# colopl/libpoporon

Measured on AMD Instinct MI355X. Metric: RS(255,223) codewords/s (encode; decode @ t=16 errs) and GB/s vs HBM peak, 1/2/4/8 GPU, higher is better.
Workload: dtype u8; 1 GPU; RS(255,223) round trip: encode + decode with 16 errors per codeword, 1048576 codewords per GPU (BASELINE configs[1]+[2]); codewords_per_gpu=1048576, layout=255-byte codeword rows, stride 255, code=poporon_config_rs_default (8, 0x11D, fcr 1, prim 1, 32 roots)

## Files before the change

### libpoporon_amd/csrc/rs_fast.hip

```cpp
#include <hip/hip_runtime.h>

#include <type_traits>

#include "rs_device.h"
#include "rs_gfa.h"
#include "rs_lane.h"

#define FWG 1024
#define NL 17
#define BWG 512
#define BM_WAVES 4

#define FAST_ROUNDS 8
static int fast_grid(size_t count, int num_cu)
{
    const size_t need = (count + FWG - 1) / FWG;
    const size_t g = FAST_ROUNDS * 2u * (size_t)(num_cu > 0 ? num_cu : 256);
    return (int)(need < g ? (need ? need : 1) : g);
}


template <bool NRG>
__global__ __launch_bounds__(BWG, BM_WAVES) void rs_bm_k(const RsDevTables *__restrict__ T, const uint8_t *__restrict__ syn,
                                                   size_t count, uint8_t *__restrict__ lamo, uint8_t *__restrict__ omo,
                                                   uint8_t *__restrict__ meta, uint32_t *__restrict__ list,
                                                   uint32_t *__restrict__ nlist, uint8_t *__restrict__ ok,
                                                   uint8_t *__restrict__ corrected, uint32_t npar)
{
    __shared__ uint32_t lgf[512 * 32];
    fill_gfa<BWG>(lgf, T);
    __syncthreads();
    const GfA gf{lds_addr(lgf) + 4u * (threadIdx.x & 31u) + 1u};
    const uint32_t pofs = gf.pofs;
    const uint32_t AZ = gf.az();
    constexpr uint32_t DQZ = SZ;

    for (size_t base = (size_t)blockIdx.x * BWG; base < count; base += (size_t)gridDim.x * BWG) {
        const size_t cw = base + threadIdx.x;
        const bool valid = cw < count;
        const uint32_t *sp = reinterpret_cast<const uint32_t *>(syn + (valid ? cw : 0) * RS_NR);
        uint4 sa = make_uint4(0, 0, 0, 0), sb = sa;
        if (valid) {
            sa = reinterpret_cast<const uint4 *>(sp)[0];
            sb = reinterpret_cast<const uint4 *>(sp)[1];
        }
        const bool any = (sa.x | sa.y | sa.z | sa.w | sb.x | sb.y | sb.z | sb.w) != 0u;
        if (__ballot(any) == 0ull) {
            if (valid) {
                ok[cw] = 1;
                if (corrected)
                    corrected[cw] = 0;
                meta[cw] = (uint8_t)(RS_ST_DONE << 5);
            }
            continue;
        }

        const uint32_t HZ = pofs + 1u;
        uint32_t hl[NL], B[NL + 1];
        hl[0] = HZ + 128u;
#pragma unroll
        for (int i = 1; i < NL; ++i)
            hl[i] = HZ;
        B[0] = pofs;
#pragma unroll
        for (int k = 1; k <= NL; ++k)
            B[k] = AZ;
        uint32_t dl = 0, db = 0, L = 0, lb = 0, ubp = 0;
        uint32_t over = 0, bo = 0;
        uint32_t WL[20];
#pragma unroll
        for (int k = 0; k < 20; ++k)
            WL[k] = SZ;
        uint32_t snext = any ? sa.x : 0u;

        auto step = [&](auto sc, uint32_t r) __attribute__((always_inline)) {
            constexpr int s = decltype(sc)::value;
            const uint32_t ub = ubp;
            uint32_t la[NL];
            uint32_t disc = 0;
            la[0] = pofs;
#pragma unroll
            for (int g = 0; g < NL; g += 4) {
#pragma unroll
                for (int i = g; i < g + 4 && i < NL; ++i)
                    if (i > 0)
                        la[i] = AZ;
                if ((uint32_t)g <= ub) {
#pragma unroll
                    for (int i = g; i < g + 4 && i < NL; ++i) {
                        if (i > 0)
                            la[i] = lds16(hl[i]);
                        disc ^= gf.expa(la[i] + WL[3 - s + i]);
                    }
                }
            }
            const uint32_t ld = gf.logs(disc);
            const bool upd = disc != 0u;
            const bool lengthen = upd && (2u * L <= r - 1u);
            const int32_t dd = (int32_t)ld - (int32_t)lb;
            const uint32_t dq = upd ? (uint32_t)(dd < 0 ? dd + 255 * 128 : dd) : DQZ;
            const uint32_t b16 = B[NL - 1] != AZ;
            over |= upd ? (bo | b16) : 0u;
            bo = lengthen ? 0u : (bo | b16);
            const uint32_t up = min((uint32_t)(NL - 1), max(dl, db + 1u));
            const uint32_t ub2 = wave_max_full(up);
            ubp = ub2;
            const uint64_t lmask = __ballot(lengthen);
            static_for<0, (NL - 1) / 4 + 1, 1>([&](auto mc) __attribute__((always_inline)) {
                constexpr int m = (NL - 1) / 4 - decltype(mc)::value;
                if ((uint32_t)(4 * m) <= ub2) {
#pragma unroll
                    for (int i = 4 * m + 3; i >= 4 * m; --i)
                        if (i > 0 && i < NL)
                            hl[i] ^= shl7(gf.expa(dq + B[i - 1]));
                    if constexpr (4 * m + 3 < NL) {
                        const uint32_t b0 = m > 0 ? B[m > 0 ? 4 * m - 1 : 0] : AZ;
                        asm("s_mov_b64 vcc, %8\n\t"
                            "v_cndmask_b32_e32 %3, %2, %7, vcc\n\t"
                            "v_cndmask_b32_e32 %2, %1, %6, vcc\n\t"
                            "v_cndmask_b32_e32 %1, %0, %5, vcc\n\t"
                            "v_cndmask_b32_e32 %0, %9, %4, vcc"
                            : "+v"(B[4 * m]), "+v"(B[4 * m + 1]), "+v"(B[4 * m + 2]), "+v"(B[4 * m + 3])
                            : "v"(la[4 * m]), "v"(la[4 * m + 1]), "v"(la[4 * m + 2]), "v"(la[4 * m + 3]),
                              "s"(lmask), "v"(b0)
                            : "vcc");
                    } else {
                        B[4 * m] = lengthen ? la[4 * m] : B[4 * m - 1];
                    }
                }
            });
            db = lengthen ? dl : min(db + 1u, (uint32_t)(NL - 1));
            if (upd)
                dl = up;
            if (lengthen) {
                L = r - L;
                lb = ld;
            }
        };
        const uint32_t nq = NRG ? (npar + 3u) >> 2 : RS_NR / 4;
#pragma unroll 1
        for (uint32_t q = 0; q < nq; ++q) {
            const uint32_t sd = snext;
            if (q + 1u < nq)
                snext = any ? sp[q + 1u] : 0u;
            const uint32_t s0 = gf.logs(sd & 0xffu), s1 = gf.logs((sd >> 8) & 0xffu);
            const uint32_t s2 = gf.logs((sd >> 16) & 0xffu), s3 = gf.logs(sd >> 24);
#pragma unroll
            for (int k = 19; k >= 4; --k)
                WL[k] = WL[k - 4];
            WL[0] = s3, WL[1] = s2, WL[2] = s1, WL[3] = s0;
            step(std::integral_constant<int, 0>{}, 4u * q + 1u);
            if (!NRG || 4u * q + 2u <= npar)
                step(std::integral_constant<int, 1>{}, 4u * q + 2u);
            if (!NRG || 4u * q + 3u <= npar)
                step(std::integral_constant<int, 2>{}, 4u * q + 3u);
            if (!NRG || 4u * q + 4u <= npar)
                step(std::integral_constant<int, 3>{}, 4u * q + 4u);
        }

        uint32_t al[NL];
        al[0] = pofs;
#pragma unroll
        for (int i = 1; i < NL; ++i)
            al[i] = (uint32_t)i <= ubp ? lds16(hl[i]) : AZ;
        uint32_t deg = 0;
#pragma unroll
        for (int i = 0; i < NL; ++i)
            deg = (al[i] & 1u) ? (uint32_t)i : deg;
        const bool fast = any && !over && deg == L && deg != 0u && (!NRG || 2u * L <= npar);

        uint32_t ob[4] = {0xFFFFFFFFu, 0xFFFFFFFFu, 0xFFFFFFFFu, 0xFFFFFFFFu};
        const uint32_t degmax = wave_max(fast ? deg : 0u);
        if (degmax) {
            const uint4 s4 = any ? reinterpret_cast<const uint4 *>(sp)[0] : make_uint4(0, 0, 0, 0);
            const uint32_t sw[4] = {s4.x, s4.y, s4.z, s4.w};
            auto omega = [&](auto dmc) __attribute__((always_inline)) {
                constexpr int DM = decltype(dmc)::value;
                uint32_t sl[16];
#pragma unroll
                for (int k = 0; k < 16; ++k)
                    sl[k] = gf.logs((sw[k >> 2] >> (8 * (k & 3))) & 0xffu);
#pragma unroll
                for (int m = 0; m < 16; ++m) {
                    if (DM ? m < DM : (uint32_t)m < degmax) {
                        uint32_t acc = 0;
#pragma unroll
                        for (int j = 0; j <= m; ++j)
                            acc ^= gf.expa(al[j] + sl[m - j]);
                        const uint32_t o = (uint32_t)m < deg ? gf.plog(gf.loga(acc)) : 255u;
                        ob[m >> 2] ^= (o ^ 0xffu) << (8 * (m & 3));
                    }
                    __builtin_amdgcn_sched_barrier(0);
                }
            };
            if (degmax == 16u)
                omega(std::integral_constant<int, 16>{});
            else
                omega(std::integral_constant<int, 0>{});
        }

        if (valid) {
            if (!any) {
                ok[cw] = 1;
                if (corrected)
                    corrected[cw] = 0;
                meta[cw] = (uint8_t)(RS_ST_DONE << 5);
            } else if (!fast) {
                meta[cw] = (uint8_t)(RS_ST_LIST << 5);
                list[atomicAdd(nlist, 1u)] = (uint32_t)cw;
            } else {
                uint32_t lb4[4] = {0, 0, 0, 0};
#pragma unroll
                for (int j = 1; j < NL; ++j)
                    lb4[(j - 1) >> 2] |= gf.plog(al[j]) << (8 * ((j - 1) & 3));
                reinterpret_cast<uint4 *>(lamo)[cw] = make_uint4(lb4[0], lb4[1], lb4[2], lb4[3]);
                reinterpret_cast<uint4 *>(omo)[cw] = make_uint4(ob[0], ob[1], ob[2], ob[3]);
                meta[cw] = (uint8_t)((RS_ST_FAST << 5) | deg);
            }
        }
    }
}




__device__ __forceinline__ uint32_t root_point(uint32_t e)
{
    return (e & 0xE0u) + 28u + ((e >> 3) & 3u) - 4u * (e & 7u);
}

__global__ __launch_bounds__(FWG, 8) void rs_chien_k(const RsDevTables *__restrict__ T, RsCorrParams P, size_t count,
                                                      const uint8_t *__restrict__ lam, uint8_t *__restrict__ meta,
                                                      uint8_t *__restrict__ roots, uint8_t *__restrict__ ok,
                                                      uint8_t *__restrict__ corrected)
{
    __shared__ uint4 lch[256 * 16];
    __shared__ uint4 lroot[FWG];
    {
        constexpr int K = 256 * 16 / FWG;
        uint4 v[K];
#pragma unroll
        for (int k = 0; k < K; ++k) {
            const uint32_t t = threadIdx.x + k * FWG;
            v[k] = T->chien[(t & 15u) * 256u + (t >> 4)];
        }
#pragma unroll
        for (int k = 0; k < K; ++k)
            lch[threadIdx.x + k * FWG] = v[k];
    }
    __syncthreads();
    const uint32_t cb = lds_addr(lch);
    const uint32_t lr0 = threadIdx.x & 15u;
    constexpr uint32_t WRAP = 255u * 256u;

    for (size_t base = (size_t)blockIdx.x * FWG; base < count; base += (size_t)gridDim.x * FWG) {
        const size_t cw = base + threadIdx.x;
        const bool valid = cw < count;
        const uint32_t st = valid ? meta[cw] : 0u;
        const bool fast = (st >> 5) == RS_ST_FAST;
        if (__ballot(fast) == 0ull)
            continue;
        const uint32_t deg = fast ? (st & 31u) : 0u;
        uint4 l4 = make_uint4(0xFFFFFFFFu, 0xFFFFFFFFu, 0xFFFFFFFFu, 0xFFFFFFFFu);
        if (fast)
            l4 = reinterpret_cast<const uint4 *>(lam)[cw];
        uint32_t lr = lr0;
        asm volatile("" : "+v"(lr));
        uint32_t D[4] = {l4.x, l4.y, l4.z, l4.w};
        uint32_t E[4];
#pragma unroll
        for (int k = 0; k < 4; ++k)
            E[k] = (lr & 4u) ? D[(k + 1) & 3] : D[k];
#pragma unroll
        for (int k = 0; k < 4; ++k)
            D[k] = (lr & 8u) ? E[(k + 2) & 3] : E[k];
        uint32_t R[4];
#pragma unroll
        for (int k = 0; k < 4; ++k)
            R[k] = __builtin_amdgcn_alignbyte(D[(k + 1) & 3], D[k], lr & 3u);
        uint32_t A[16], inc[16];
#pragma unroll
        for (int k = 0; k < 16; ++k) {
            const uint32_t jm = ((uint32_t)k + lr) & 15u;
            const uint32_t e = (R[k >> 2] >> (8 * (k & 3))) & 0xffu;
            A[k] = cb + (e << 8) + (jm << 4);
            inc[k] = e == 255u ? WRAP : (jm == 15u ? 256u : (jm + 1u) << 12);
        }
        lroot[threadIdx.x] = make_uint4(0, 0, 0, 0);
        uint32_t lp = lds_addr(lroot) + 16u * threadIdx.x;
        uint32_t cnt = 0, z0 = 0;
        auto push = [&](uint32_t v) __attribute__((always_inline)) {
            lds_st8(lp, v);
            lp += 1u;
        };
#pragma unroll 1
        for (int w = 0; w < 8; ++w) {
            uint32_t word = 0;
#pragma unroll
            for (int h = 0; h < 2; ++h) {
                uint32_t acc[4] = {0x01010101u, 0x01010101u, 0x01010101u, 0x01010101u};
#pragma unroll
                for (int k = 0; k < 16; k += 2) {
                    const lds_u32x4_t r1 = lds128(A[k]), r2 = lds128(A[k + 1]);
                    A[k] = chien_step<WRAP>(A[k], inc[k]);
                    A[k + 1] = chien_step<WRAP>(A[k + 1], inc[k + 1]);
                    acc[0] = xor3(acc[0], r1.x, r2.x);
                    acc[1] = xor3(acc[1], r1.y, r2.y);
                    acc[2] = xor3(acc[2], r1.z, r2.z);
                    acc[3] = xor3(acc[3], r1.w, r2.w);
                }
#pragma unroll
                for (int d = 0; d < 4; ++d)
                    word = __builtin_amdgcn_bitop3_b32(word, zero80(acc[d]) >> (d + 4 * h), 0u, 0xF0 | 0xCC);
            }
            if (w == 7)
                word &= ~(1u << 24);
            if (w == 0) {
                z0 = (word >> 7) & 1u;
                word &= ~0x80u;
            }
            cnt += __popc(word);
            const uint32_t wb = 32u * (uint32_t)w;
            while (word != 0u) {
                const uint32_t b = __builtin_ctz(word);
                word &= word - 1u;
                push(wb | b);
            }
        }
        if (z0)
            push(248u);
        cnt += z0;
        const uint4 l4r = lroot[threadIdx.x];
        const uint32_t L[4] = {l4r.x, l4r.y, l4r.z, l4r.w};
        bool good = cnt == deg;
        if (P.pad > 0) {
            bool low = false;
#pragma unroll
            for (int n = 0; n < 16; ++n) {
                const uint32_t i = root_point((L[n >> 2] >> (8 * (n & 3))) & 0xffu);
                low |= (uint32_t)n < cnt && (int32_t)((i * P.iprim + 254u) % 255u) < P.pad;
            }
            good = good && !low;
        }
        if (fast)
            reinterpret_cast<uint4 *>(roots)[2 * cw] = make_uint4(L[0], L[1], L[2], L[3]);
        if (fast && !good) {
            {
                ok[cw] = 0;
                if (corrected)
                    corrected[cw] = 0;
                meta[cw] = (uint8_t)(RS_ST_DONE << 5);
            }
        }
    }
}


#ifndef F2WG
#define F2WG 1024
#endif
#ifndef F2_WAVES
#define F2_WAVES (F2WG / 128)
#endif
#ifndef FORNEY_R
#define FORNEY_R 2
#endif
template <bool P11>
__global__ __launch_bounds__(F2WG, F2_WAVES) void rs_forney_k(const RsDevTables *__restrict__ T, RsCorrParams P,
                                                      uint8_t *data, size_t dstride, uint8_t *parity, size_t pstride,
                                                      size_t count, const uint8_t *__restrict__ lam,
                                                      const uint8_t *__restrict__ om, uint8_t *__restrict__ roots,
                                                      const uint8_t *__restrict__ meta, uint8_t *__restrict__ ok,
                                                      uint8_t *__restrict__ corrected)
{
    __shared__ uint32_t lgf[512 * 32];
    fill_gfa<F2WG>(lgf, T);
    __syncthreads();
    const GfA gf{lds_addr(lgf) + 4u * (threadIdx.x & 31u) + 1u};
    const int32_t pad = P.pad;
    constexpr bool fcr1 = P11, iprim1 = P11;
    constexpr int R = FORNEY_R;
    const uint32_t mp = 255u * 128u + gf.pofs;

    for (size_t base = (size_t)blockIdx.x * F2WG; base < count; base += (size_t)gridDim.x * F2WG) {
        const size_t cw = base + threadIdx.x;
        const bool valid = cw < count;
        const uint32_t st = valid ? meta[cw] : 0u;
        const bool fast = (st >> 5) == RS_ST_FAST;
        if (__ballot(fast) == 0ull)
            continue;
        const uint32_t deg = fast ? (st & 31u) : 0u;
        uint4 o4 = make_uint4(0xFFFFFFFFu, 0xFFFFFFFFu, 0xFFFFFFFFu, 0xFFFFFFFFu), l4 = o4;
        uint32_t rl[4] = {0, 0, 0, 0};
        if (fast) {
            o4 = reinterpret_cast<const uint4 *>(om)[cw];
            l4 = reinterpret_cast<const uint4 *>(lam)[cw];
            const uint4 ra = reinterpret_cast<const uint4 *>(roots)[2 * cw];
            rl[0] = ra.x, rl[1] = ra.y, rl[2] = ra.z, rl[3] = ra.w;
        }
        const uint32_t ow[4] = {o4.x, o4.y, o4.z, o4.w}, lw[4] = {l4.x, l4.y, l4.z, l4.w};
        const uint32_t dtop = deg ? (deg - 1u) & ~1u : 0u;
        uint32_t opu[16], lod[8];
#pragma unroll
        for (int m = 0; m < 16; ++m)
            opu[m] = gf.afrom((ow[m >> 2] >> (8 * (m & 3))) & 0xffu);
#pragma unroll
        for (int h = 0; h < 8; ++h)
            lod[h] = (uint32_t)(2 * h) <= dtop ? gf.afrom((lw[(2 * h) >> 2] >> (8 * ((2 * h) & 3))) & 0xffu) : gf.az();
        const uint32_t degmax = wave_max(deg);
        uint32_t posp[4] = {0, 0, 0, 0}, magp[4] = {0, 0, 0, 0};
        uint32_t fixed = 0;
#pragma unroll
        for (int n0 = 0; n0 < 16; n0 += R) {
            if ((uint32_t)n0 >= degmax)
                continue;
            uint32_t ir[R], si[R], s[R], num[R], den[R], nh[R], dh[R];
#pragma unroll
            for (int t = 0; t < R; ++t) {
                ir[t] = root_point((rl[(n0 + t) >> 2] >> (8 * ((n0 + t) & 3))) & 0xffu);
                si[t] = 128u * (ir[t] == 255u ? 0u : ir[t]);
                s[t] = num[t] = den[t] = nh[t] = dh[t] = 0;
            }
#pragma unroll
            for (int b = 0; b < 8; ++b) {
#pragma unroll
                for (int t = 0; t < R; ++t) {
                    num[t] ^= gf.expa(opu[b] + s[t]);
                    nh[t] ^= gf.expa(opu[b + 8] + s[t]);
                    if ((b & 1) == 0) {
                        den[t] ^= gf.expa(lod[b >> 1] + s[t]);
                        dh[t] ^= gf.expa(lod[(b >> 1) + 4] + s[t]);
                    }
                    s[t] = addmod7(s[t], si[t]);
                }
                if (b & 1) {
#pragma unroll
                    for (int t = 0; t < R; ++t)
                        asm volatile("" : "+v"(num[t]), "+v"(den[t]), "+v"(nh[t]), "+v"(dh[t]));
                    __builtin_amdgcn_sched_barrier(0);
                }
            }
#pragma unroll
            for (int t = 0; t < R; ++t) {
                num[t] ^= gf.expa(gf.loga(nh[t]) + s[t]);
                den[t] ^= gf.expa(gf.loga(dh[t]) + s[t]);
                uint32_t mag;
                if constexpr (fcr1) {
                    mag = gf.expa(gf.loga(num[t]) - gf.loga(den[t]) + mp);
                } else {
                    const uint32_t ln2 = mod255((uint32_t)((int32_t)ir[t] * ((int32_t)P.fcr - 1) + (int32_t)RS_NN));
                    const uint32_t lden = gf.plog(gf.loga(den[t]));
                    mag = gf.exp(red(gf.plog(gf.loga(num[t])) + ln2 + RS_NN - lden));
                }
                const bool z = (uint32_t)(n0 + t) < deg && num[t] != 0u;
                fixed += z ? 1u : 0u;
                const uint32_t k = iprim1 ? ir[t] - 1u : (ir[t] * P.iprim + 254u) % 255u;
                const uint32_t p = (uint32_t)((int32_t)k - pad);
                posp[(n0 + t) >> 2] |= (p & 0xffu) << (8 * ((n0 + t) & 3));
                magp[(n0 + t) >> 2] |= (z ? mag : 0u) << (8 * ((n0 + t) & 3));
            }
            __builtin_amdgcn_sched_barrier(0);
        }
        if (fast) {
            uint4 *rec = reinterpret_cast<uint4 *>(roots + cw * 32u);
            rec[0] = make_uint4(posp[0], posp[1], posp[2], posp[3]);
            rec[1] = make_uint4(magp[0], magp[1], magp[2], magp[3]);
            ok[cw] = 1;
            if (corrected)
                corrected[cw] = (uint8_t)fixed;
        }
    }
}
// ... 875 lines not shown
```

### libpoporon_amd/csrc/rs_lane.h

```cpp
#ifndef POPORON_AMD_RS_LANE_H
#define POPORON_AMD_RS_LANE_H

#include <hip/hip_runtime.h>

#include "rs_device.h"

typedef __attribute__((address_space(3))) const uint8_t lds_u8;
typedef __attribute__((address_space(3))) const uint16_t lds_u16;
typedef unsigned lds_u32x4_t __attribute__((ext_vector_type(4)));
typedef __attribute__((address_space(3))) const lds_u32x4_t lds_u32x4;

__device__ __forceinline__ uint32_t lds8(uint32_t a) { return *(lds_u8 *)(size_t)a; }
__device__ __forceinline__ uint32_t lds16(uint32_t a) { return *(lds_u16 *)(size_t)a; }
__device__ __forceinline__ lds_u32x4_t lds128(uint32_t a) { return *(lds_u32x4 *)(size_t)a; }
__device__ __forceinline__ void lds_st8(uint32_t a, uint32_t v)
{
    *(__attribute__((address_space(3))) uint8_t *)(size_t)a = (uint8_t)v;
}
template <typename T> __device__ __forceinline__ uint32_t lds_addr(const T *p)
{
    return (uint32_t)(size_t)(__attribute__((address_space(3))) const T *)p;
}

__device__ __forceinline__ uint32_t mod255(uint32_t v) { return (v & 0xffffu) % 255u; }
__device__ __forceinline__ uint32_t red(uint32_t x) { return min(x, x - 255u); }
__device__ __forceinline__ uint32_t conv(uint32_t s8)
{
    return (uint32_t)max((int32_t)s8, ((int32_t)s8 - 254) * 1024);
}

__device__ __forceinline__ uint32_t half(const uint32_t *a, int i)
{
    return (i & 1) ? (a[i >> 1] >> 16) : (a[i >> 1] & 0xffffu);
}

__device__ __forceinline__ uint32_t addmod7(uint32_t x, uint32_t y)
{
    uint32_t t, u, r;
    asm("v_add_u16 %0, %1, %2" : "=v"(t) : "v"(x), "v"(y));
    asm("v_subrev_u16 %0, 0x7f80, %1" : "=v"(u) : "v"(t));
    asm("v_min_u16 %0, %1, %2" : "=v"(r) : "v"(t), "v"(u));
    return r;
}

__device__ __forceinline__ void prio_by_progress(uint32_t it)
{
    switch (it) {
    case 0: __builtin_amdgcn_s_setprio(3); break;
    case 1: __builtin_amdgcn_s_setprio(2); break;
    case 2: __builtin_amdgcn_s_setprio(1); break;
    default: __builtin_amdgcn_s_setprio(0); break;
    }
}

template <uint32_t WRAP>
__device__ __forceinline__ uint32_t chien_step(uint32_t a, uint32_t inc)
{
    uint32_t t1, t2, r;
    asm("v_add_u32_e32 %0, %3, %4\n\t"
        "v_subrev_co_u32_e32 %1, vcc, %5, %0\n\t"
        "v_cndmask_b32_e32 %2, %1, %0, vcc"
        : "=&v"(t1), "=&v"(t2), "=v"(r)
        : "v"(a), "v"(inc), "i"(WRAP)
        : "vcc");
    return r;
}

__device__ __forceinline__ uint32_t xor3(uint32_t a, uint32_t b, uint32_t c)
{
    return __builtin_amdgcn_bitop3_b32(a, b, c, 0x96);
}

__device__ __forceinline__ uint32_t wave_max(uint32_t v)
{
    uint32_t m = 0;
#pragma unroll
    for (int b = 5; b >= 0; --b) {
        const uint32_t c = m | (1u << b);
        if (__ballot(v >= c) != 0ull)
            m = c;
    }
    return m;
}

__device__ __forceinline__ uint32_t wave_min(uint32_t v) { return 63u - wave_max(63u - v); }

__device__ __forceinline__ uint32_t wave_max_full(uint32_t v)
{
    uint32_t x = v;
    x = max(x, (uint32_t)__builtin_amdgcn_update_dpp(0, (int)x, 0x111, 0xf, 0xf, true));
    x = max(x, (uint32_t)__builtin_amdgcn_update_dpp(0, (int)x, 0x112, 0xf, 0xf, true));
    x = max(x, (uint32_t)__builtin_amdgcn_update_dpp(0, (int)x, 0x114, 0xf, 0xf, true));
    x = max(x, (uint32_t)__builtin_amdgcn_update_dpp(0, (int)x, 0x118, 0xf, 0xf, true));
    x = max(x, (uint32_t)__builtin_amdgcn_update_dpp(0, (int)x, 0x142, 0xa, 0xf, false));
    x = max(x, (uint32_t)__builtin_amdgcn_update_dpp(0, (int)x, 0x143, 0xc, 0xf, false));
    return __builtin_amdgcn_readlane(x, 63);
}

__device__ __forceinline__ uint32_t zero80(uint32_t v)
{
    const uint32_t t = (v & 0x7F7F7F7Fu) + 0x7F7F7F7Fu;
    return __builtin_amdgcn_bitop3_b32(t, v, 0x7F7F7F7Fu, 0x01);
}

__device__ __forceinline__ uint32_t zero_bytes16(const uint32_t (&v)[4])
{
    uint32_t m = 0;
#pragma unroll
    for (int d = 0; d < 4; ++d) {
        const uint32_t z = ~(((v[d] & 0x7F7F7F7Fu) + 0x7F7F7F7Fu) | v[d] | 0x7F7F7F7Fu);
        const uint32_t t = (z >> 7) & 0x01010101u;
        m |= ((t * 0x10204080u) >> 28) << (4 * d);
    }
    return m;
}

struct RootIter {
    uint32_t w[9];
    __device__ __forceinline__ void init(const uint32_t (&rb)[8])
    {
#pragma unroll
        for (int k = 0; k < 8; ++k)
            w[k] = rb[k];
        w[8] = rb[0] & 1u;
        w[0] &= ~1u;
    }
    __device__ __forceinline__ uint32_t next()
    {
        uint32_t sel = 8, bits = w[8];
#pragma unroll
        for (int k = 7; k >= 0; --k) {
            const bool nz = w[k] != 0u;
            sel = nz ? (uint32_t)k : sel;
            bits = nz ? w[k] : bits;
        }
        const uint32_t b = __builtin_ctz(bits | 0x80000000u);
        const uint32_t clr = bits & (bits - 1u);
#pragma unroll
        for (int k = 0; k < 9; ++k)
            w[k] = (sel == (uint32_t)k) ? clr : w[k];
        return sel < 8u ? 32u * sel + b : 255u;
    }
};

#endif
```

Measured before the change: 2.224 billion codewords/s.

## Replace per-step wave-max reduction in Berlekamp-Massey with ballot-based bound tracking

Reworks the Berlekamp-Massey step so the active-degree bound grows by at most one per step through a single ballot, instead of a full DPP wave-max reduction and readlane. Per-lane control state (update flag, lengthen, overflow tracking) moves into wave-wide ballot masks. Conditional register updates become cndmask sequences, L is stored doubled, and the discrepancy log and difference use 16-bit LDS and modular helpers. The aim is fewer cross-lane reductions and VALU instructions per step, at the cost of a looser bound that may evaluate more polynomial terms (the added script counts how many).

```diff
diff --git a/libpoporon_amd/csrc/rs_fast.hip b/libpoporon_amd/csrc/rs_fast.hip
--- a/libpoporon_amd/csrc/rs_fast.hip
+++ b/libpoporon_amd/csrc/rs_fast.hip
@@ -65,8 +65,8 @@
 #pragma unroll
         for (int k = 1; k <= NL; ++k)
             B[k] = AZ;
-        uint32_t dl = 0, db = 0, L = 0, lb = 0, ubp = 0;
-        uint32_t over = 0, bo = 0;
+        uint32_t dl = 0, D = 1, L2 = 0, lbp = pofs, ubp = 0;
+        uint64_t overm = 0, bom = 0;
         uint32_t WL[20];
 #pragma unroll
         for (int k = 0; k < 20; ++k)
@@ -81,10 +81,6 @@
             la[0] = pofs;
 #pragma unroll
             for (int g = 0; g < NL; g += 4) {
-#pragma unroll
-                for (int i = g; i < g + 4 && i < NL; ++i)
-                    if (i > 0)
-                        la[i] = AZ;
                 if ((uint32_t)g <= ub) {
 #pragma unroll
                     for (int i = g; i < g + 4 && i < NL; ++i) {
@@ -94,25 +90,44 @@
                     }
                 }
             }
-            const uint32_t ld = gf.logs(disc);
-            const bool upd = disc != 0u;
-            const bool lengthen = upd && (2u * L <= r - 1u);
-            const int32_t dd = (int32_t)ld - (int32_t)lb;
-            const uint32_t dq = upd ? (uint32_t)(dd < 0 ? dd + 255 * 128 : dd) : DQZ;
-            const uint32_t b16 = B[NL - 1] != AZ;
-            over |= upd ? (bo | b16) : 0u;
-            bo = lengthen ? 0u : (bo | b16);
-            const uint32_t up = min((uint32_t)(NL - 1), max(dl, db + 1u));
-            const uint32_t ub2 = wave_max_full(up);
+            const uint32_t ld = lds16(HZ + shl7(disc));
+            const uint64_t updm = __ballot(disc != 0u);
+            const uint64_t lmask = updm & __ballot(L2 < r);
+            const uint64_t b16m = bom | __ballot(B[NL - 1] != AZ);
+            overm |= updm & b16m;
+            bom = b16m & ~lmask;
+            const uint32_t cD = min16_u16(D);
+            const uint32_t up = max_u16(dl, cD);
+            const uint32_t ub2 = ub + (__ballot(up > ub) != 0ull ? 1u : 0u);
             ubp = ub2;
-            const uint64_t lmask = __ballot(lengthen);
+            const uint32_t dq0 = submod7(ld, lbp);
+            const uint32_t nl2 = 2u * r - L2;
+            uint32_t dq, dn;
+            asm("s_mov_b64 vcc, %[lm]\n\t"
+                "v_cndmask_b32_e32 %[dn], %[cd], %[dl], vcc\n\t"
+                "v_cndmask_b32_e32 %[l2], %[l2], %[nl2], vcc\n\t"
+                "v_cndmask_b32_e32 %[lbp], %[lbp], %[ld], vcc\n\t"
+                "s_mov_b64 vcc, %[um]\n\t"
+                "v_cndmask_b32_e32 %[dq], %[dqz], %[dq0], vcc\n\t"
+                "v_cndmask_b32_e32 %[dl], %[dl], %[up], vcc"
+                : [dn] "=&v"(dn), [l2] "+v"(L2), [lbp] "+v"(lbp), [dq] "=&v"(dq), [dl] "+v"(dl)
+                : [cd] "v"(cD), [nl2] "v"(nl2), [ld] "v"(ld), [dq0] "v"(dq0), [up] "v"(up), [dqz] "v"(DQZ),
+                  [lm] "s"(lmask), [um] "s"(updm)
+                : "vcc");
+            D = dn + 1u;
             static_for<0, (NL - 1) / 4 + 1, 1>([&](auto mc) __attribute__((always_inline)) {
                 constexpr int m = (NL - 1) / 4 - decltype(mc)::value;
+                const uint64_t lm = lmask;
                 if ((uint32_t)(4 * m) <= ub2) {
 #pragma unroll
                     for (int i = 4 * m + 3; i >= 4 * m; --i)
                         if (i > 0 && i < NL)
                             hl[i] ^= shl7(gf.expa(dq + B[i - 1]));
+                    if ((uint32_t)(4 * m) > ub) {
+#pragma unroll
+                        for (int i = 4 * m; i < 4 * m + 4 && i < NL; ++i)
+                            la[i] = AZ;
+                    }
                     if constexpr (4 * m + 3 < NL) {
                         const uint32_t b0 = m > 0 ? B[m > 0 ? 4 * m - 1 : 0] : AZ;
                         asm("s_mov_b64 vcc, %8\n\t"
@@ -122,20 +137,17 @@
                             "v_cndmask_b32_e32 %0, %9, %4, vcc"
                             : "+v"(B[4 * m]), "+v"(B[4 * m + 1]), "+v"(B[4 * m + 2]), "+v"(B[4 * m + 3])
                             : "v"(la[4 * m]), "v"(la[4 * m + 1]), "v"(la[4 * m + 2]), "v"(la[4 * m + 3]),
-                              "s"(lmask), "v"(b0)
+                              "s"(lm), "v"(b0)
                             : "vcc");
                     } else {
-                        B[4 * m] = lengthen ? la[4 * m] : B[4 * m - 1];
+                        asm("s_mov_b64 vcc, %3\n\t"
+                            "v_cndmask_b32_e32 %0, %1, %2, vcc"
+                            : "=v"(B[4 * m])
+                            : "v"(B[4 * m - 1]), "v"(la[4 * m]), "s"(lm)
+                            : "vcc");
                     }
                 }
             });
-            db = lengthen ? dl : min(db + 1u, (uint32_t)(NL - 1));
-            if (upd)
-                dl = up;
-            if (lengthen) {
-                L = r - L;
-                lb = ld;
-            }
         };
         const uint32_t nq = NRG ? (npar + 3u) >> 2 : RS_NR / 4;
 #pragma unroll 1
@@ -167,7 +179,8 @@
 #pragma unroll
         for (int i = 0; i < NL; ++i)
             deg = (al[i] & 1u) ? (uint32_t)i : deg;
-        const bool fast = any && !over && deg == L && deg != 0u && (!NRG || 2u * L <= npar);
+        const bool over = (overm >> (threadIdx.x & 63u)) & 1ull;
+        const bool fast = any && !over && 2u * deg == L2 && deg != 0u && (!NRG || L2 <= npar);
 
         uint32_t ob[4] = {0xFFFFFFFFu, 0xFFFFFFFFu, 0xFFFFFFFFu, 0xFFFFFFFFu};
         const uint32_t degmax = wave_max(fast ? deg : 0u);
diff --git a/libpoporon_amd/csrc/rs_lane.h b/libpoporon_amd/csrc/rs_lane.h
--- a/libpoporon_amd/csrc/rs_lane.h
+++ b/libpoporon_amd/csrc/rs_lane.h
@@ -40,6 +40,28 @@
     asm("v_add_u16 %0, %1, %2" : "=v"(t) : "v"(x), "v"(y));
     asm("v_subrev_u16 %0, 0x7f80, %1" : "=v"(u) : "v"(t));
     asm("v_min_u16 %0, %1, %2" : "=v"(r) : "v"(t), "v"(u));
+    return r;
+}
+
+__device__ __forceinline__ uint32_t submod7(uint32_t x, uint32_t y)
+{
+    uint32_t t, u, r;
+    asm("v_sub_u16 %0, %1, %2" : "=v"(t) : "v"(x), "v"(y));
+    asm("v_add_u16 %0, 0x7f80, %1" : "=v"(u) : "v"(t));
+    asm("v_min_u16 %0, %1, %2" : "=v"(r) : "v"(t), "v"(u));
+    return r;
+}
+
+__device__ __forceinline__ uint32_t min16_u16(uint32_t a)
+{
+    uint32_t r;
+    asm("v_min_u16 %0, 16, %1" : "=v"(r) : "v"(a));
+    return r;
+}
+__device__ __forceinline__ uint32_t max_u16(uint32_t a, uint32_t b)
+{
+    uint32_t r;
+    asm("v_max_u16 %0, %1, %2" : "=v"(r) : "v"(a), "v"(b));
     return r;
 }
 
diff --git a/profiles/experiments/bm_guard_terms.py b/profiles/experiments/bm_guard_terms.py
--- /dev/null
+++ b/profiles/experiments/bm_guard_terms.py
@@ -0,0 +1,10 @@
+#!/usr/bin/env python3
+
+
+def terms(bound):
+    return sum(min(17, 4 * (bound(r) // 4) + 4) for r in range(1, 33))
+
+
+exact = terms(lambda r: min(16, (r + 1) // 2))
+by_r = terms(lambda r: min(16, r))
+print(f"exact wave maximum: {exact} terms; bound min(16, r): {by_r} terms (+{100 * (by_r - exact) / exact:.0f} %)")
```

Result: faster. 2.261 billion codewords/s, median of 6 (+1.6%).
